# sz3/libcimbar

Hardware: NVIDIA H100
Metric: decoded cimbar frames/sec (1024x1024 mode-B) (higher is better)
Workload: dtype u8 (integer/bitwise; float32 only in the colour classifier, bit-exact vs reference)

## Files before the change

### libcimbar_b200/csrc/api.cu

```cuda
#include "ctx.cuh"
#include "k1_decode.cuh"
#include "k2_rs.cuh"
#include "render.cuh"
#include "encode.cuh"

#include <atomic>
#include <cmath>
#include <cstdio>
#include <cstring>
#include <string>
#include <vector>

using namespace cb200;

namespace {

thread_local std::string g_err;
std::atomic<unsigned long long> g_launches{0};

}
namespace cb200 {
int fail(int code, const std::string& msg) { g_err = msg; return code; }
int fail_cuda(cudaError_t e, const char* what)
{
// ... 393 lines not shown
    CK(cudaStreamCreateWithFlags(&c->own_stream, cudaStreamNonBlocking), "cudaStreamCreate");
    c->stream = c->own_stream;

    float adjust[256];
    adjust[0] = 0.0f;
    for (int d = 1; d < 256; ++d) adjust[d] = (float)(255.0 / (double)(float)d);
    unsigned long long tilesL[16];
    for (int t = 0; t < 16; ++t) tilesL[t] = brev64(kTilesH[t]);
    CK(k1_init_tables(adjust, tilesL), "k1 tables");
    CK(render_init_tables(kTilesH), "render tables");
    uint8_t gexp[512], glog[256];
    {
        unsigned el = 1; gexp[0] = 1; glog[0] = 0;
        for (unsigned i = 1; i < 512; ++i) {
            el *= 2; if (el > 255) el ^= 0x187u;
            gexp[i] = (uint8_t)el;
            if (i < 256) glog[el] = (uint8_t)i;
        }
    }
    CK(k2_init_tables(gexp, glog), "k2 tables");
    CK(flood_init_tables(adjust, tilesL, m.hash_mul), "flood tables");

    size_t n = (size_t)max_frames;
    CK(c->d_cellvals.ensure(n * m.num_cells), "cudaMalloc cellvals");
    CK(c->d_dirty.ensure(n), "cudaMalloc dirty");
    CK(c->d_raw.ensure(n * m.cap_all + 16), "cudaMalloc raw");
    CK(c->d_data.ensure(n * m.data_bytes), "cudaMalloc data");
    CK(c->d_ok.ensure(n * m.nblocks), "cudaMalloc ok");
    CK(c->d_mask.ensure(n), "cudaMalloc mask");
    CK(c->d_flags.ensure(n), "cudaMalloc flags");
    std::vector<uint16_t> idx;
    interleave_indices(m, idx);
    CK(c->d_idx.ensure(idx.size()), "cudaMalloc idx");
    CK(cudaMemcpy(c->d_idx, idx.data(), idx.size() * sizeof(uint16_t), cudaMemcpyHostToDevice), "upload idx");
    {
        std::vector<uint16_t> inv(idx.size());
        for (size_t sidx = 0; sidx < idx.size(); ++sidx) inv[idx[sidx]] = (uint16_t)sidx;
        CK(c->d_inv.ensure(inv.size()), "cudaMalloc inv");
        CK(cudaMemcpy(c->d_inv, inv.data(), inv.size() * sizeof(uint16_t), cudaMemcpyHostToDevice), "upload inv");
        std::vector<uint8_t> g(1, 1);
        auto mul = [&](uint8_t a, uint8_t b) -> uint8_t { return (a && b) ? gexp[glog[a] + glog[b]] : 0; };
        for (int i = 1; i <= m.ecc_bytes; ++i) {
            uint8_t root = gexp[i % 255];
            std::vector<uint8_t> ng(g.size() + 1, 0);
            for (size_t k = 0; k < g.size(); ++k) { ng[k + 1] ^= g[k]; ng[k] ^= mul(g[k], root); }
            g.swap(ng);
        }
        CK(c->d_gen.ensure(g.size()), "cudaMalloc gen");
        CK(cudaMemcpy(c->d_gen, g.data(), g.size(), cudaMemcpyHostToDevice), "upload gen");
        uint8_t rho[4 * 64];
        k2_remainder_basis(g.data(), m.ecc_bytes, gexp, glog, rho);
        CK(c->d_rho.ensure(sizeof(rho)), "cudaMalloc rho");
        CK(cudaMemcpy(c->d_rho, rho, sizeof(rho), cudaMemcpyHostToDevice), "upload rho");
        CK(encode_init_tables(gexp, glog), "encode tables");
    }
    {
        std::vector<uint16_t> adj;
        build_adjacency(m, adj);
        if (!adjacency_consistent(m, adj)) return fail(CB200_ERR_MODE, "adjacency self-check failed");
        CK(flood_workspace_create(m, c->sm_count, adj.data(), &c->flood), "flood workspace");
    }
    return CB200_OK;
}

int cb200_create(cb200_ctx** out, int device, int mode_val, int max_frames)
{
    if (!out || max_frames < 1) return fail(CB200_ERR_ARG, "bad arguments");
    *out = nullptr;
    int ndev = 0;
    if (cudaGetDeviceCount(&ndev) != cudaSuccess || ndev == 0)
        return fail(CB200_ERR_NODEVICE, "no CUDA device: libcb200 has no CPU fallback");
    if (device < 0) { CK(cudaGetDevice(&device), "cudaGetDevice"); }
    if (device >= ndev) return fail(CB200_ERR_ARG, "device index out of range");
    CK(cudaSetDevice(device), "cudaSetDevice");
    cb200_ctx* c = new cb200_ctx();
    c->device = device;
    int rc = create_impl(c, device, mode_val, max_frames);
    if (rc != CB200_OK) {
        std::string why = cb200_last_error();
        cb200_destroy(c);
        return fail(rc, why);
    }
    *out = c;
    return CB200_OK;
}

int cb200_destroy(cb200_ctx* c)
{
    if (!c) return CB200_OK;
    cudaSetDevice(c->device);
    for (int k = 0; k < cb200_ctx::kEvSets; ++k) for (int i = 0; i < 8; ++i) if (c->ev[k][i]) cudaEventDestroy(c->ev[k][i]);
    for (const auto& s : c->stage) if (s.ev) cudaEventDestroy(s.ev);
    if (c->ccm_ev) cudaEventDestroy(c->ccm_ev);
    gather_destroy(c->gather);
    deskew_destroy(c->deskew); scan_destroy(c->scan);
    if (c->own_stream) cudaStreamDestroy(c->own_stream);
    delete c;
    return CB200_OK;
}

int cb200_get_info(const cb200_ctx* c, cb200_info* out)
{
    if (!c || !out) return fail(CB200_ERR_ARG, "null argument");
    fill_info(c->mode, c->max_frames, c->sm_count, out);
    return CB200_OK;
}
// ... 4 lines not shown
    c->stream = cuda_stream ? (cudaStream_t)cuda_stream : c->own_stream;
    return CB200_OK;
}

int cb200_sync(cb200_ctx* c)
{
    if (!c) return fail(CB200_ERR_ARG, "null context");
    CK(cudaStreamSynchronize(c->stream), "cudaStreamSynchronize");
    return CB200_OK;
}

int cb200_decode_raw_dev(cb200_ctx* c, const uint8_t* d_rgb, int n, uint32_t flags, uint8_t* d_raw_out, uint8_t* d_frame_flags)
{
    int rc = check_frame_flags(flags); if (rc) return rc;
    rc = check_n(c, n); if (rc) return rc;
    if (n == 0) return CB200_OK;
    if (!d_rgb || !d_raw_out) return fail(CB200_ERR_ARG, "null buffer");
    CK(cudaSetDevice(c->device), "cudaSetDevice");
    const uint16_t* idx;
    rc = idx_for(c, flags, &idx); if (rc) return rc;
    rc = run_cells(c, d_rgb, n, flags, nullptr); if (rc) return rc;
    CK(k2_pack_launch(c->mode, c->d_cellvals, idx, n, d_raw_out, c->stream), "pack launch");
    mark(c);
    if (d_frame_flags) CK(cudaMemcpyAsync(d_frame_flags, c->d_flags, (size_t)n, cudaMemcpyDeviceToDevice, c->stream), "copy flags");
    return CB200_OK;
}

int cb200_rs_correct_dev(cb200_ctx* c, const uint8_t* d_raw, int n, uint8_t* d_data_out, uint8_t* d_block_ok)
{
    int rc = check_n(c, n); if (rc) return rc;
    if (n == 0) return CB200_OK;
    if (!d_raw || !d_data_out) return fail(CB200_ERR_ARG, "null buffer");
    CK(cudaSetDevice(c->device), "cudaSetDevice");
    uint8_t* ok = d_block_ok ? d_block_ok : c->d_ok;
    CK(k2_rs_launch(c->mode, d_raw, n, d_data_out, ok, c->d_rho, c->sm_count, c->stream), "rs launch");
    return CB200_OK;
}

}

namespace {
int decode_chunks(cb200_ctx* c, const uint8_t* d_rgb, int n, uint32_t flags, const uint8_t* sharpen, uint8_t* d_chunks,
                  uint32_t* d_chunk_mask, uint8_t* d_frame_flags)
{
    int rc = check_n(c, n); if (rc) return rc;
    if (n == 0) return CB200_OK;
    if (!d_rgb || !d_chunks || !d_chunk_mask) return fail(CB200_ERR_ARG, "null buffer");
    CK(cudaSetDevice(c->device), "cudaSetDevice");
    const Mode& m = c->mode;
    if ((flags & CB200_FLAG_CC_FIT) && (flags & CB200_FLAG_CC_SIMPLE)) return fail(CB200_ERR_ARG, "CC_SIMPLE and CC_FIT are exclusive");
    const bool fit = (flags & CB200_FLAG_CC_FIT) && !m.legacy && m.ecc_bytes > 0 && m.color_bits > 0;
    const uint16_t* idx;
    rc = idx_for(c, flags, &idx); if (rc) return rc;
    if (!fit) {
        rc = run_cells(c, d_rgb, n, flags & ~CB200_FLAG_CC_FIT, sharpen); if (rc) return rc;
        mark(c);
        CK(k2_rs_fused_launch(m, c->d_cellvals, idx, n, d_chunks, c->d_ok, c->d_rho, c->sm_count, c->stream), "rs launch");
    } else {
        rc = ccm_buffers(c); if (rc) return rc;
        CK(c->d_means.ensure((size_t)c->max_frames * m.num_cells), "cudaMalloc means");
        CK(c->d_ccm_active.ensure((size_t)c->max_frames), "cudaMalloc ccm flags");
        CcmArg initial;
        rc = ccm_arg(c, initial); if (rc) return rc;
        rc = run_cells(c, d_rgb, n, flags & ~(CB200_FLAG_CC_FIT | CB200_FLAG_CC_SIMPLE), sharpen, nullptr, c->d_means); if (rc) return rc;
        mark(c);
        CK(k2_rs_fused_launch(m, c->d_cellvals, idx, n, d_chunks, c->d_ok, c->d_rho, c->sm_count, c->stream, 0, m.nblocks_sym), "rs launch (symbols)");
        CK(ccm_fit_launch(m, d_rgb, d_chunks, c->d_ok, idx, n, c->d_fit, c->d_fit_valid, c->stream), "ccm fit");
        CK(ccm_carry_launch(n, c->d_fit, c->d_fit_valid, initial, c->d_ccm, c->d_ccm_active, c->stream), "ccm carry");
        CK(ccm_apply_launch(m, c->d_means, n, c->d_ccm, c->d_ccm_active, c->d_cellvals, c->stream), "ccm apply");
        CK(k2_rs_fused_launch(m, c->d_cellvals, idx, n, d_chunks, c->d_ok, c->d_rho, c->sm_count, c->stream, m.nblocks_sym, m.nblocks - m.nblocks_sym),
           "rs launch (colours)");
        rc = ccm_keep_last(c, n, c->d_ccm_active); if (rc) return rc;
    }
    mark(c);
    CK(k2_mask_launch(m, c->d_ok, n, d_chunk_mask, c->stream), "mask launch");
    mark(c);
    if (d_frame_flags) CK(cudaMemcpyAsync(d_frame_flags, c->d_flags, (size_t)n, cudaMemcpyDeviceToDevice, c->stream), "copy flags");
    return CB200_OK;
}
}

extern "C" {

int cb200_decode_chunks_dev(cb200_ctx* c, const uint8_t* d_rgb, int n, uint32_t flags, uint8_t* d_chunks, uint32_t* d_chunk_mask, uint8_t* d_frame_flags)
{
    int rc = check_frame_flags(flags); if (rc) return rc;
    return decode_chunks(c, d_rgb, n, flags, nullptr, d_chunks, d_chunk_mask, d_frame_flags);
}

int cb200_decode_chunks_sharpen_dev(cb200_ctx* c, const uint8_t* d_rgb, int n, uint32_t flags, const uint8_t* sharpen, uint8_t* d_chunks,
                                    uint32_t* d_chunk_mask, uint8_t* d_frame_flags)
{
    int rc = check_selection_args(flags, sharpen); if (rc) return rc;
    return decode_chunks(c, d_rgb, n, flags, sharpen, d_chunks, d_chunk_mask, d_frame_flags);
}

int cb200_decode_raw(cb200_ctx* c, const uint8_t* rgb, int n, uint32_t flags, uint8_t* raw_out, uint8_t* frame_flags)
{
    int rc = check_frame_flags(flags); if (rc) return rc;
    rc = check_n(c, n); if (rc) return rc;
    if (n == 0) return CB200_OK;
    if (!rgb || !raw_out) return fail(CB200_ERR_ARG, "null buffer");
    CK(cudaSetDevice(c->device), "cudaSetDevice");
    rc = upload_frames(c, rgb, n); if (rc) return rc;
    rc = cb200_decode_raw_dev(c, c->d_rgb, n, flags, c->d_raw, nullptr); if (rc) return rc;
    CK(cudaMemcpyAsync(raw_out, c->d_raw, (size_t)n * c->mode.cap_all, cudaMemcpyDeviceToHost, c->stream), "D2H raw");
    if (frame_flags) CK(cudaMemcpyAsync(frame_flags, c->d_flags, (size_t)n, cudaMemcpyDeviceToHost, c->stream), "D2H flags");
    CK(cudaStreamSynchronize(c->stream), "sync");
    return CB200_OK;
}

int cb200_decode(cb200_ctx* c, const uint8_t* rgb, int n, uint32_t flags, uint8_t* data_out, uint8_t* block_ok, uint8_t* frame_flags)
{
    int rc = check_frame_flags(flags); if (rc) return rc;
    rc = check_n(c, n); if (rc) return rc;
    if (n == 0) return CB200_OK;
    if (!rgb || !data_out) return fail(CB200_ERR_ARG, "null buffer");
    CK(cudaSetDevice(c->device), "cudaSetDevice");
    rc = upload_frames(c, rgb, n); if (rc) return rc;
    rc = cb200_decode_chunks_dev(c, c->d_rgb, n, flags, c->d_data, c->d_mask, nullptr); if (rc) return rc;
    CK(cudaMemcpyAsync(data_out, c->d_data, (size_t)n * c->mode.data_bytes, cudaMemcpyDeviceToHost, c->stream), "D2H data");
    if (block_ok) CK(cudaMemcpyAsync(block_ok, c->d_ok, (size_t)n * c->mode.nblocks, cudaMemcpyDeviceToHost, c->stream), "D2H ok");
    if (frame_flags) CK(cudaMemcpyAsync(frame_flags, c->d_flags, (size_t)n, cudaMemcpyDeviceToHost, c->stream), "D2H flags");
// ... 238 lines not shown
```

### libcimbar_b200/csrc/ctx.cuh

```cuda
#pragma once
#include "../../include/cb200.h"
#include "cb200_common.cuh"
#include "k1x_flood.cuh"
#include "ccm.cuh"

#include <string>
#include <vector>

namespace cb200 {
int fail(int code, const std::string& msg);
int fail_cuda(cudaError_t e, const char* what);
struct GatherState;
struct DeskewState;
struct ScanScratch;
void gather_destroy(GatherState* g);
void deskew_destroy(DeskewState* d);
void scan_destroy(ScanScratch* s);
int decode_fountain_to_host(cb200_ctx* c, const uint8_t* d_rgb, int n, uint32_t flags, const uint8_t* sharpen, uint8_t* chunks_out,
                            uint32_t* chunk_count, uint32_t* chunk_mask, uint8_t* frame_flags);
int check_camera_flags(uint32_t flags);
struct PicDesc {
    uint64_t src;
    uint64_t blur;
    int w, h;
    int words;
    int tile0;
};
int check_picture_sizes(const int32_t* wh, int n);
std::vector<int32_t> uniform_sizes(int w, int h, int n);
int extract_decode_to_host(cb200_ctx* c, const uint8_t* d_src, const int32_t* wh, int n, const float* corners, uint32_t flags,
                           const uint8_t* sharpen, uint8_t* chunks_out, uint32_t* chunk_count, uint32_t* chunk_mask, uint8_t* frame_flags);
std::vector<uint8_t> sharpen_from_corners(const cb200_ctx* c, const float* corners, int n);
}
#define CK(call, what) do { cudaError_t e__ = (call); if (e__ != cudaSuccess) return cb200::fail_cuda(e__, what); } while (0)

struct cb200_ctx {
    cb200::Mode mode;
    int device = 0, max_frames = 0, sm_count = 0;
    cudaStream_t own_stream = nullptr, stream = nullptr;
    cb200::DevBuf<uint8_t> d_rgb;
    cb200::DevBuf<uint8_t> d_cellvals;
    cb200::DevBuf<uint32_t> d_dirty;
    cb200::DevBuf<uint8_t> d_raw;
    cb200::DevBuf<uint8_t> d_data;
    cb200::DevBuf<uint8_t> d_ok;
    cb200::DevBuf<uint32_t> d_mask;
    cb200::DevBuf<uint8_t> d_flags;
    cb200::DevBuf<uint16_t> d_idx;
    cb200::DevBuf<uint16_t> d_inv;
    cb200::DevBuf<uint16_t> d_idx_ident;
    cb200::DevBuf<uint8_t> d_gen;
    cb200::DevBuf<uint8_t> d_rho;
    bool timing = false;
    static constexpr int kEvSets = 64;
    cudaEvent_t ev[kEvSets][8] = {};
    int ev_count[kEvSets] = {};
    long calls = 0;
    int cur = 0;
    cb200::FloodWorkspace flood;
    cb200::DevBuf<uint8_t> d_scratch;
    cb200::PinnedBuf<uint8_t> h_pinned;
    struct StageSlot { cb200::PinnedBuf<uint8_t> h; cudaEvent_t ev = nullptr; };
    static constexpr int kStageSlots = 3;
    StageSlot stage[kStageSlots];
    int stage_next = 0;
    cb200::DevBuf<uint8_t> d_sel;
    float ccm[9] = {};
    bool ccm_active = false;
    bool ccm_pending = false;
    bool ccm_pending_flag = false;
    cb200::DevBuf<float> d_ccm;
    cb200::PinnedBuf<float> h_ccm;
    cb200::DevBuf<uint32_t> d_means;
    cb200::DevBuf<float> d_fit;
    cb200::DevBuf<uint8_t> d_fit_valid;
    cb200::DevBuf<uint8_t> d_ccm_active;
    cudaEvent_t ccm_ev = nullptr;
    cb200::GatherState* gather = nullptr;
    cb200::DeskewState* deskew = nullptr;
    cb200::ScanScratch* scan = nullptr;
};

namespace cb200 {
inline void begin_timed_call(cb200_ctx* c) { if (c->timing) { c->cur = (int)(c->calls % cb200_ctx::kEvSets); c->calls++; c->ev_count[c->cur] = 0; } }
inline void mark(cb200_ctx* c) { if (c->timing && c->ev_count[c->cur] < 8) cudaEventRecord(c->ev[c->cur][c->ev_count[c->cur]++], c->stream); }
int stage_take(cb200_ctx* c, size_t bytes, int* slot, uint8_t** h);
int stage_send(cb200_ctx* c, int slot, void* d_dst, size_t bytes, const char* what);
}
```

### libcimbar_b200/csrc/k2_rs.cu

```cuda
#include "cb200_common.cuh"
#include "k2_rs.cuh"
#include <cstring>
#include <cstdint>

namespace cb200 {

constexpr int kMaxParity = 64;

__constant__ uint8_t c_gf_exp[512];
__constant__ uint8_t c_gf_log[256];

__device__ __forceinline__ uint32_t slot_value(const uint8_t* __restrict__ cells, const uint16_t* __restrict__ idx,
                                               uint32_t s, int stream, int symbol_bits)
{
    uint32_t v = cells[idx[s]] & 0x7Fu;
    uint32_t sym_mask = (1u << symbol_bits) - 1u;
    if (stream == 0) return v & sym_mask;
    if (stream == 1) return v >> symbol_bits;
    return v;
}

__device__ __forceinline__ uint32_t stream_byte(const uint8_t* __restrict__ cells, const uint16_t* __restrict__ idx,
                                                uint32_t B, int w, int stream, int symbol_bits, uint32_t nslots)
{
// ... 347 lines not shown
                }
            } else {
                const uint8_t* enc_g = raw + (size_t)f * m.cap_all + (size_t)b * blk;
                for (int i = lane; i < blk; i += 32) enc[i] = enc_g[i];
            }
        }
        __syncwarp();

        uint32_t word = 0;
        {
            const int top_src = grp * GL + (Pw - 1);
#pragma unroll 2
            for (int t = 0; t < nsteps; ++t) {
                const uint32_t ew = lds_u32(stage_lane + 4u * (uint32_t)t);
                const uint32_t tw = __shfl_sync(0xffffffffu, word, top_src);
                const uint32_t v = tw ^ __byte_perm(ew, 0u, 0x0123);
                const uint32_t r0 = lds_u32(lt_lane + (((v) & 0xFFu) + 0u) * (4u * GL));
                const uint32_t r1 = lds_u32(lt_lane + (((v >> 8) & 0xFFu) + 256u) * (4u * GL));
                const uint32_t r2 = lds_u32(lt_lane + (((v >> 16) & 0xFFu) + 512u) * (4u * GL));
                const uint32_t r3 = lds_u32(lt_lane + ((v >> 24) + 768u) * (4u * GL));
                uint32_t prev = __shfl_up_sync(0xffffffffu, word, 1, GL);
                if (k == 0) prev = 0;
                word = prev ^ r0 ^ r1 ^ r2 ^ r3;
            }
        }
        const uint32_t dirty = __ballot_sync(0xffffffffu, k < Pw && word != 0u);

#pragma unroll 1
        for (int g = 0; g < G; ++g) {
            const long gb = unit * G + g;
            if (gb >= total_blocks) break;
            const int f = (int)(gb / b_count), b = b_begin + (int)(gb - (long)f * b_count);
            uint8_t* out = data_out + ((size_t)f * m.nblocks + b) * msg_len;
            uint8_t* enc = w.stage + g * kStagePitch + lead;
            if (((dirty >> (g * GL)) & ((1u << GL) - 1u)) == 0u) {
                for (int i = lane; i < msg_len; i += 32) out[i] = enc[i];
                if (lane == 0) block_ok[(size_t)f * m.nblocks + b] = 1;
                continue;
            }
            __syncwarp();
            const bool good = rs_correct_block<T>(s, w, enc, md, blk, pad, grp == g && k < Pw, word, k, lane);
            __syncwarp();
            if (!good) {
                for (int i = lane; i < msg_len; i += 32) out[i] = 0;
                if (lane == 0) block_ok[(size_t)f * m.nblocks + b] = 0;
                continue;
            }
        for (int i = lane; i < msg_len; i += 32) out[i] = enc[i];
        if (lane == 0) block_ok[(size_t)f * m.nblocks + b] = 1;
        }
    }
}

constexpr int kFrWarps = 32;
constexpr int kFrFrames = 2;
constexpr int kFrBlk = 155, kFrWords = 39, kFrPitch = 160;

struct RsFrSmem {
    static constexpr bool kSynTable = true;
    uint8_t exp[512];
    uint8_t log[256];
    struct PerWarp {
        alignas(8) uint2 masks[32];
        alignas(4) uint8_t rem[64];
        alignas(2) uint16_t remlog[kMaxParity];
        uint8_t synd[kMaxParity];
        uint8_t loc[kMaxParity + 8];
        uint8_t last[kMaxParity + 8];
        uint8_t omega[kMaxParity];
        uint8_t roots[kMaxParity + 8];
    } w[kFrWarps];
    uint8_t la[kLaDim][kLaDim];
    alignas(8) uint2 wsyn[32][32];
};

__device__ __forceinline__ void cp_async16(uint32_t dst_shared, const void* src)
{
    asm volatile("cp.async.cg.shared.global [%0], [%1], 16;" ::"r"(dst_shared), "l"(src) : "memory");
}

__global__ void __launch_bounds__(kFrWarps * 32, 2)
k_rs_frames(const Mode m, const uint8_t* __restrict__ cellvals, const uint16_t* __restrict__ idx, int n_frames,
            uint8_t* __restrict__ data_out, uint8_t* __restrict__ block_ok, const uint8_t* __restrict__ rho, int cell_pitch)
{
    constexpr int GL = 8, G = 4;
    extern __shared__ __align__(16) uint8_t rs_smem_raw[];
    RsFrSmem& s = *reinterpret_cast<RsFrSmem*>(rs_smem_raw);
    uint8_t* dyn = rs_smem_raw + ((sizeof(RsFrSmem) + 127) & ~size_t(127));
    uint32_t* lt = reinterpret_cast<uint32_t*>(dyn);
    uint8_t* cellbuf = dyn + sizeof(uint32_t) * 4 * 256 * GL;
    uint8_t* rows = cellbuf + (size_t)kFrFrames * cell_pitch;
    const int tid = threadIdx.x, warp = tid >> 5, lane = tid & 31;
    const int md = m.ecc_bytes, msg_len = m.msg_len, nb = m.nblocks, upf = nb / G;
    const int Pw = (md + 3) >> 2, pad = 4 * Pw - md;
    const int words_per_frame = nb * kFrWords, sym_rows = m.cap_sym / kFrBlk, cell_vecs = m.num_cells >> 4;
    const bool coupled6 = m.legacy != 0;
    const int n_groups = (n_frames + kFrFrames - 1) / kFrFrames;
    const uint32_t cellbuf_s = (uint32_t)__cvta_generic_to_shared(cellbuf);

    auto load_cells = [&](int gi) {
        for (int fs = 0; fs < kFrFrames; ++fs) {
            const int f = gi * kFrFrames + fs;
            if (f >= n_frames) break;
            const uint8_t* src = cellvals + (size_t)f * m.num_cells;
            for (int i = tid; i < cell_vecs; i += (int)blockDim.x) cp_async16(cellbuf_s + (uint32_t)(fs * cell_pitch + 16 * i), src + 16 * i);
        }
        asm volatile("cp.async.commit_group;" ::: "memory");
    };
    int gi = blockIdx.x;
    if (gi < n_groups) load_cells(gi);

    for (int i = tid; i < 512; i += blockDim.x) s.exp[i] = c_gf_exp[i];
    for (int i = tid; i < 256; i += blockDim.x) s.log[i] = c_gf_log[i];
    __syncthreads();
    for (int e = tid; e < md * kLaDim; e += blockDim.x) {
        const int kk = e / kLaDim, j = e % kLaDim;
        s.la[kk][j] = (uint8_t)((255 - ((j + 1) * (md - kk)) % 255) % 255);
    }
    for (int e = tid; e < 32 * 32; e += blockDim.x) {
        const int i = e >> 5, j = e & 31;
        uint2 t = make_uint2(0u, 0u);
        if (i < md && j < md) {
            const uint32_t l = (uint32_t)((255 - ((j + 1) * (md - i)) % 255) % 255);
            t.x = (uint32_t)s.exp[l] | ((uint32_t)s.exp[l + 1] << 8) | ((uint32_t)s.exp[l + 2] << 16) | ((uint32_t)s.exp[l + 3] << 24);
            t.y = (uint32_t)s.exp[l + 4] | ((uint32_t)s.exp[l + 5] << 8) | ((uint32_t)s.exp[l + 6] << 16) | ((uint32_t)s.exp[l + 7] << 24);
        }
        s.wsyn[i][j] = t;
    }
    for (int e = tid; e < 4 * 256 * GL; e += blockDim.x) {
        const int v = e / (4 * GL), j = (e / GL) & 3, kk = e % GL;
        uint32_t word = 0;
#pragma unroll
        for (int bb = 0; bb < 4; ++bb) word |= gf_mul(s, (uint32_t)v, (uint32_t)rho[j * 64 + 4 * kk + bb]) << (8 * bb);
        lt[e] = word;
    }

    RsFrSmem::PerWarp& w = s.w[warp];
    const int grp = lane / GL, k = lane % GL;
    const uint32_t lt_lane = (uint32_t)__cvta_generic_to_shared(lt) + 4u * (uint32_t)k;
    const uint32_t vsel = 0x3210u ^ (0x1111u * (uint32_t)grp);
    const uint32_t lt0 = lt_lane + 32u * (uint32_t)(0 ^ grp), lt1 = lt_lane + 32u * (uint32_t)(1 ^ grp);
    const uint32_t lt2 = lt_lane + 32u * (uint32_t)(2 ^ grp), lt3 = lt_lane + 32u * (uint32_t)(3 ^ grp);

    for (; gi < n_groups; gi += gridDim.x) {
        asm volatile("cp.async.wait_all;" ::: "memory");
        __syncthreads();
        const int nf = (n_frames - gi * kFrFrames) < kFrFrames ? (n_frames - gi * kFrFrames) : kFrFrames;

        for (int wi = tid; wi < nf * words_per_frame; wi += (int)blockDim.x) {
            const int fs = wi >= words_per_frame ? 1 : 0;
            const int rem = wi - fs * words_per_frame;
            const int r = rem / kFrWords, q = rem - r * kFrWords;
            const uint8_t* cb = cellbuf + fs * cell_pitch;
            uint32_t b0, b1, b2, b3;
            if (coupled6) {
                auto byte6 = [&](const int B) -> uint32_t {
                    const uint32_t bit0 = 8u * (uint32_t)B, sl = bit0 / 6u, skip = bit0 - 6u * sl;
                    const uint32_t v0 = cb[idx[sl]] & 63u, v1 = cb[idx[sl + 1]] & 63u;
                    return (((v0 << 6) | v1) >> (4u - skip)) & 0xFFu;
                };
                const int B0 = r * kFrBlk + 4 * q - 1;
                b0 = q ? byte6(B0) : 0u; b1 = byte6(B0 + 1); b2 = byte6(B0 + 2); b3 = byte6(B0 + 3);
            } else if (r < sym_rows) {
                const uint32_t* ix = reinterpret_cast<const uint32_t*>(idx) + (r * kFrBlk + 4 * q);
                const uint32_t i0 = q ? ix[-1] : ix[0], i1 = ix[0], i2 = ix[1], i3 = ix[2];
                b0 = ((cb[i0 & 0xFFFFu] & 15u) << 4) | (cb[i0 >> 16] & 15u);
                b1 = ((cb[i1 & 0xFFFFu] & 15u) << 4) | (cb[i1 >> 16] & 15u);
                b2 = ((cb[i2 & 0xFFFFu] & 15u) << 4) | (cb[i2 >> 16] & 15u);
                b3 = ((cb[i3 & 0xFFFFu] & 15u) << 4) | (cb[i3 >> 16] & 15u);
            } else {
                const uint2* ix = reinterpret_cast<const uint2*>(idx) + ((r - sym_rows) * kFrBlk + 4 * q);
                const uint2 i0 = q ? ix[-1] : ix[0], i1 = ix[0], i2 = ix[1], i3 = ix[2];
                auto pack = [&](const uint2 ii) {
                    return (((uint32_t)cb[ii.x & 0xFFFFu] >> 4) & 3u) << 6 | (((uint32_t)cb[ii.x >> 16] >> 4) & 3u) << 4 |
                           (((uint32_t)cb[ii.y & 0xFFFFu] >> 4) & 3u) << 2 | (((uint32_t)cb[ii.y >> 16] >> 4) & 3u);
                };
                b0 = pack(i0); b1 = pack(i1); b2 = pack(i2); b3 = pack(i3);
            }
            if (q == 0) b0 = 0;
            *reinterpret_cast<uint32_t*>(rows + (size_t)(fs * nb + r) * kFrPitch + 4 * q) = b0 | (b1 << 8) | (b2 << 16) | (b3 << 24);
        }
        __syncthreads();
        if (gi + (int)gridDim.x < n_groups) load_cells(gi + (int)gridDim.x);

        if (warp >= nf * upf) continue;
        const int fs = warp >= upf ? 1 : 0, u = warp - fs * upf, f = gi * kFrFrames + fs;
        uint8_t* urow = rows + (size_t)(fs * nb + G * u) * kFrPitch;

        uint32_t word = 0;
        {
            const uint32_t stage_lane = (uint32_t)__cvta_generic_to_shared(urow) + (uint32_t)(grp * kFrPitch);
            const int top_src = grp * GL + (Pw - 1);
#pragma unroll 3
            for (int t = 0; t < kFrWords; ++t) {
                const uint32_t ew = lds_u32(stage_lane + 4u * (uint32_t)t);
                const uint32_t tw = __shfl_sync(0xffffffffu, word, top_src);
                const uint32_t v = __byte_perm(tw ^ __byte_perm(ew, 0u, 0x0123), 0u, vsel);
                const uint32_t r0 = lds_u32(lt0 + ((v) & 0xFFu) * 128u);
                const uint32_t r1 = lds_u32(lt1 + ((v >> 8) & 0xFFu) * 128u);
                const uint32_t r2 = lds_u32(lt2 + ((v >> 16) & 0xFFu) * 128u);
                const uint32_t r3 = lds_u32(lt3 + (v >> 24) * 128u);
                uint32_t prev = __shfl_up_sync(0xffffffffu, word, 1, GL);
                if (k == 0) prev = 0;
                word = prev ^ r0 ^ r1 ^ r2 ^ r3;
            }
        }
        const uint32_t dirty = __ballot_sync(0xffffffffu, k < Pw && word != 0u);
        uint32_t okflags = 0x01010101u;
        if (dirty) {
#pragma unroll 1
            for (int g = 0; g < G; ++g) {
                if (((dirty >> (g * GL)) & ((1u << GL) - 1u)) == 0u) continue;
                uint8_t* enc = urow + g * kFrPitch + 1;
                __syncwarp();
                const bool good = rs_correct_block<1>(s, w, enc, md, kFrBlk, pad, grp == g && k < Pw, word, k, lane);
                __syncwarp();
                if (!good) {
                    for (int i = lane; i < msg_len; i += 32) enc[i] = 0;
                    okflags &= ~(1u << (8 * g));
                }
            }
            __syncwarp();
        }
        uint32_t* out32 = reinterpret_cast<uint32_t*>(data_out + ((size_t)f * nb + (size_t)(G * u)) * msg_len);
        const uint32_t urow_s = (uint32_t)__cvta_generic_to_shared(urow);
        for (int wq = lane; wq < msg_len; wq += 32) {
            const int B = 4 * wq;
            int g = (B >= msg_len) + (B >= 2 * msg_len) + (B >= 3 * msg_len);
            int i = B - g * msg_len;
            uint32_t val;
            if (i + 4 <= msg_len) {
                const uint32_t a = (uint32_t)(g * kFrPitch + 1 + i);
                const uint32_t w0 = lds_u32(urow_s + (a & ~3u)), w1 = lds_u32(urow_s + (a & ~3u) + 4u);
                val = __funnelshift_r(w0, w1, 8u * (a & 3u));
            } else {
                val = 0;
#pragma unroll
                for (int j = 0; j < 4; ++j) {
                    val |= (uint32_t)urow[g * kFrPitch + 1 + i] << (8 * j);
                    if (++i == msg_len) { i = 0; ++g; }
                }
            }
            out32[wq] = val;
// ... 10 lines not shown
    uint32_t out = 0;
    bool carry = false;
    for (int q = 0; q < m.chunks_per_frame; ++q) {
        bool all = true;
        for (int k = 0; k < m.blocks_per_chunk; ++k) all = all && (ok[q * m.blocks_per_chunk + k] != 0);
        if (all && !carry) out |= 1u << q;
        carry = ok[q * m.blocks_per_chunk + m.blocks_per_chunk - 1] == 0;
    }
    mask[f] = out;
}

cudaError_t k2_init_tables(const uint8_t* exp512, const uint8_t* log256)
{
    cudaError_t e = cudaMemcpyToSymbol(c_gf_exp, exp512, 512);
    if (e != cudaSuccess) return e;
    return cudaMemcpyToSymbol(c_gf_log, log256, 256);
}

cudaError_t k2_pack_launch(const Mode& m, const uint8_t* d_cellvals, const uint16_t* d_idx, int n_frames, uint8_t* d_raw, cudaStream_t st)
{
    dim3 grid((m.cap_all + 255) / 256, n_frames);
    k_pack_raw<<<grid, 256, 0, st>>>(m, d_cellvals, d_idx, n_frames, d_raw); count_launch();
    return cudaGetLastError();
}

template <int T, bool FUSED>
static cudaError_t rs_launch_t(const Mode& m, const uint8_t* d_raw, const uint8_t* d_cellvals, const uint16_t* d_idx, int n_frames,
                               uint8_t* d_data, uint8_t* d_ok, const uint8_t* d_rho, int sm_count, cudaStream_t st, int b_begin = 0, int b_count = -1)
{
    if (b_count < 0) b_count = m.nblocks;
    if (m.ecc_block + 4 > kStagePitch || m.ecc_bytes > 8 * T * 4 || m.ecc_bytes > kLaDim) return cudaErrorInvalidValue;
    const size_t smem = ((sizeof(RsSmem<T>) + 127) & ~size_t(127)) + sizeof(uint32_t) * 4 * 256 * 8 * T;
    {
        cudaError_t e = cudaFuncSetAttribute(k_rs_decode<T, FUSED>, cudaFuncAttributeMaxDynamicSharedMemorySize, (int)smem);
        if (e != cudaSuccess) return e;
    }
    const int G = 4 / T;
    long total = (long)n_frames * b_count;
    long units = (total + G - 1) / G;
    long ctas = (units + kRsWarpsPerCta - 1) / kRsWarpsPerCta;
    long max_ctas = (long)sm_count * (T == 1 ? 4 : 2);
    if (ctas > max_ctas) ctas = max_ctas;
    if (ctas < 1) ctas = 1;
    k_rs_decode<T, FUSED><<<(int)ctas, kRsWarpsPerCta * 32, smem, st>>>(m, d_raw, d_cellvals, d_idx, n_frames, b_begin, b_count, d_data, d_ok, d_rho); count_launch();
    return cudaGetLastError();
}

cudaError_t k2_rs_launch(const Mode& m, const uint8_t* d_raw, int n_frames, uint8_t* d_data, uint8_t* d_ok, const uint8_t* d_rho, int sm_count, cudaStream_t st)
{
    if (m.ecc_bytes <= 32) return rs_launch_t<1, false>(m, d_raw, nullptr, nullptr, n_frames, d_data, d_ok, d_rho, sm_count, st);
    return rs_launch_t<2, false>(m, d_raw, nullptr, nullptr, n_frames, d_data, d_ok, d_rho, sm_count, st);
}

cudaError_t k2_rs_fused_launch(const Mode& m, const uint8_t* d_cellvals, const uint16_t* d_idx, int n_frames, uint8_t* d_data,
                               uint8_t* d_ok, const uint8_t* d_rho, int sm_count, cudaStream_t st, int b_begin, int b_count)
{
    if (b_count < 0) b_count = m.nblocks;
    const bool whole = b_begin == 0 && b_count == m.nblocks;
    const bool bits_ok = m.symbol_bits == 4 && m.color_bits == 2 && (!m.legacy || (size_t)m.num_cells * 6 == (size_t)m.cap_all * 8);
    if (whole && bits_ok && m.ecc_block == kFrBlk && m.ecc_bytes <= 32 &&
        m.ecc_bytes <= kLaDim && m.nblocks % 4 == 0 && kFrFrames * (m.nblocks / 4) <= kFrWarps && m.num_cells % 16 == 0 &&
        m.cap_sym % kFrBlk == 0 && (m.nblocks * m.msg_len) % 4 == 0 && ((uintptr_t)d_data & 3u) == 0 && n_frames > 0) {
        const int cell_pitch = m.num_cells;
        const size_t smem = ((sizeof(RsFrSmem) + 127) & ~size_t(127)) + sizeof(uint32_t) * 4 * 256 * 8 +
                            (size_t)kFrFrames * cell_pitch + (size_t)kFrFrames * m.nblocks * kFrPitch;
        if (smem <= 113 * 1024) {
            cudaError_t e = cudaFuncSetAttribute(k_rs_frames, cudaFuncAttributeMaxDynamicSharedMemorySize, (int)smem);
            if (e != cudaSuccess) return e;
            int groups = (n_frames + kFrFrames - 1) / kFrFrames, ctas = groups < 2 * sm_count ? groups : 2 * sm_count;
            k_rs_frames<<<ctas, 32 * kFrFrames * (m.nblocks / 4), smem, st>>>(m, d_cellvals, d_idx, n_frames, d_data, d_ok, d_rho, cell_pitch); count_launch();
            return cudaGetLastError();
        }
    }
    if (m.ecc_bytes <= 32) return rs_launch_t<1, true>(m, nullptr, d_cellvals, d_idx, n_frames, d_data, d_ok, d_rho, sm_count, st, b_begin, b_count);
    return rs_launch_t<2, true>(m, nullptr, d_cellvals, d_idx, n_frames, d_data, d_ok, d_rho, sm_count, st, b_begin, b_count);
}

void k2_remainder_basis(const uint8_t* gen, int parity, const uint8_t* gexp512, const uint8_t* glog256, uint8_t* rho_out )
{
    const int Pw = (parity + 3) / 4, D = 4 * Pw, pad = D - parity;
    uint8_t G[72] = {0};
    for (int k = 0; k <= parity; ++k) G[pad + k] = gen[k];
    auto mul = [&](uint8_t x, uint8_t y) -> uint8_t { return (x && y) ? gexp512[glog256[x] + glog256[y]] : 0; };
    uint8_t r[64] = {0};
    r[0] = 1;
    for (int e = 1; e <= D + 3; ++e) {
        const uint8_t top = r[D - 1];
        for (int k = D - 1; k > 0; --k) r[k] = r[k - 1];
        r[0] = 0;
        if (top) for (int k = 0; k < D; ++k) r[k] ^= mul(top, G[k]);
        if (e >= D) { for (int k = 0; k < 64; ++k) rho_out[(e - D) * 64 + k] = k < D ? r[k] : 0; }
    }
}

cudaError_t k2_mask_launch(const Mode& m, const uint8_t* d_ok, int n_frames, uint32_t* d_mask, cudaStream_t st)
{
    k_chunk_mask<<<(n_frames + 127) / 128, 128, 0, st>>>(m, d_ok, n_frames, d_mask); count_launch();
    return cudaGetLastError();
}

}
```

### libcimbar_b200/csrc/k2_rs.cuh

```cuda
#pragma once
#include "cb200_common.cuh"

namespace cb200 {
cudaError_t k2_init_tables(const uint8_t* exp512, const uint8_t* log256);
cudaError_t k2_pack_launch(const Mode& m, const uint8_t* d_cellvals, const uint16_t* d_idx, int n_frames, uint8_t* d_raw, cudaStream_t st);
cudaError_t k2_rs_launch(const Mode& m, const uint8_t* d_raw, int n_frames, uint8_t* d_data, uint8_t* d_ok, const uint8_t* d_rho, int sm_count, cudaStream_t st);
void k2_remainder_basis(const uint8_t* gen, int parity, const uint8_t* gexp512, const uint8_t* glog256, uint8_t* rho_out);
cudaError_t k2_rs_fused_launch(const Mode& m, const uint8_t* d_cellvals, const uint16_t* d_idx, int n_frames, uint8_t* d_data,
                               uint8_t* d_ok, const uint8_t* d_rho, int sm_count, cudaStream_t st, int b_begin = 0, int b_count = -1);
cudaError_t k2_mask_launch(const Mode& m, const uint8_t* d_ok, int n_frames, uint32_t* d_mask, cudaStream_t st);
}
```

Before: 901,600.

## Replace per-byte index gather with analytic interleave unpack in fused RS kernel

```diff
diff --git a/libcimbar_b200/csrc/api.cu b/libcimbar_b200/csrc/api.cu
--- a/libcimbar_b200/csrc/api.cu
+++ b/libcimbar_b200/csrc/api.cu
@@ -469,6 +469,10 @@
         k2_remainder_basis(g.data(), m.ecc_bytes, gexp, glog, rho);
         CK(c->d_rho.ensure(sizeof(rho)), "cudaMalloc rho");
         CK(cudaMemcpy(c->d_rho, rho, sizeof(rho), cudaMemcpyHostToDevice), "upload rho");
+        std::vector<uint64_t> tables((k2_frame_tables_size() + 7) / 8);
+        k2_frame_tables(gexp, glog, rho, m.ecc_bytes, tables.data());
+        CK(c->d_rs_tables.ensure(k2_frame_tables_size()), "cudaMalloc rs tables");
+        CK(cudaMemcpy(c->d_rs_tables, tables.data(), k2_frame_tables_size(), cudaMemcpyHostToDevice), "upload rs tables");
         CK(encode_init_tables(gexp, glog), "encode tables");
     }
     {
@@ -579,10 +583,11 @@
     const bool fit = (flags & CB200_FLAG_CC_FIT) && !m.legacy && m.ecc_bytes > 0 && m.color_bits > 0;
     const uint16_t* idx;
     rc = idx_for(c, flags, &idx); if (rc) return rc;
+    const bool il = !(flags & CB200_FLAG_NO_INTERLEAVE);
     if (!fit) {
         rc = run_cells(c, d_rgb, n, flags & ~CB200_FLAG_CC_FIT, sharpen); if (rc) return rc;
         mark(c);
-        CK(k2_rs_fused_launch(m, c->d_cellvals, idx, n, d_chunks, c->d_ok, c->d_rho, c->sm_count, c->stream), "rs launch");
+        CK(k2_rs_fused_launch(m, c->d_cellvals, idx, il, n, d_chunks, c->d_ok, c->d_rho, c->d_rs_tables, c->sm_count, c->stream), "rs launch");
     } else {
         rc = ccm_buffers(c); if (rc) return rc;
         CK(c->d_means.ensure((size_t)c->max_frames * m.num_cells), "cudaMalloc means");
@@ -591,11 +596,12 @@
         rc = ccm_arg(c, initial); if (rc) return rc;
         rc = run_cells(c, d_rgb, n, flags & ~(CB200_FLAG_CC_FIT | CB200_FLAG_CC_SIMPLE), sharpen, nullptr, c->d_means); if (rc) return rc;
         mark(c);
-        CK(k2_rs_fused_launch(m, c->d_cellvals, idx, n, d_chunks, c->d_ok, c->d_rho, c->sm_count, c->stream, 0, m.nblocks_sym), "rs launch (symbols)");
+        CK(k2_rs_fused_launch(m, c->d_cellvals, idx, il, n, d_chunks, c->d_ok, c->d_rho, c->d_rs_tables, c->sm_count, c->stream, 0, m.nblocks_sym), "rs launch (symbols)");
         CK(ccm_fit_launch(m, d_rgb, d_chunks, c->d_ok, idx, n, c->d_fit, c->d_fit_valid, c->stream), "ccm fit");
         CK(ccm_carry_launch(n, c->d_fit, c->d_fit_valid, initial, c->d_ccm, c->d_ccm_active, c->stream), "ccm carry");
         CK(ccm_apply_launch(m, c->d_means, n, c->d_ccm, c->d_ccm_active, c->d_cellvals, c->stream), "ccm apply");
-        CK(k2_rs_fused_launch(m, c->d_cellvals, idx, n, d_chunks, c->d_ok, c->d_rho, c->sm_count, c->stream, m.nblocks_sym, m.nblocks - m.nblocks_sym),
+        CK(k2_rs_fused_launch(m, c->d_cellvals, idx, il, n, d_chunks, c->d_ok, c->d_rho, c->d_rs_tables, c->sm_count, c->stream, m.nblocks_sym,
+                              m.nblocks - m.nblocks_sym),
            "rs launch (colours)");
         rc = ccm_keep_last(c, n, c->d_ccm_active); if (rc) return rc;
     }
diff --git a/libcimbar_b200/csrc/ctx.cuh b/libcimbar_b200/csrc/ctx.cuh
--- a/libcimbar_b200/csrc/ctx.cuh
+++ b/libcimbar_b200/csrc/ctx.cuh
@@ -51,6 +51,7 @@
     cb200::DevBuf<uint16_t> d_idx_ident;
     cb200::DevBuf<uint8_t> d_gen;
     cb200::DevBuf<uint8_t> d_rho;
+    cb200::DevBuf<uint8_t> d_rs_tables;
     bool timing = false;
     static constexpr int kEvSets = 64;
     cudaEvent_t ev[kEvSets][8] = {};
diff --git a/libcimbar_b200/csrc/k2_rs.cu b/libcimbar_b200/csrc/k2_rs.cu
--- a/libcimbar_b200/csrc/k2_rs.cu
+++ b/libcimbar_b200/csrc/k2_rs.cu
@@ -423,143 +423,183 @@
     }
 }
 
-constexpr int kFrWarps = 32;
-constexpr int kFrFrames = 2;
+constexpr int kFrWarps = 16;
 constexpr int kFrBlk = 155, kFrWords = 39, kFrPitch = 160;
-
-struct RsFrSmem {
-    static constexpr bool kSynTable = true;
+constexpr int kFrLead = 16;
+
+struct RsFrTables {
     uint8_t exp[512];
     uint8_t log[256];
+    alignas(8) uint2 wsyn[32][32];
+    uint32_t lt[4 * 256 * 8];
+};
+static_assert(sizeof(RsFrTables) % 16 == 0, "the tables are copied in 16-byte pieces");
+
+struct RsFrSmem : RsFrTables {
+    static constexpr bool kSynTable = true;
     struct PerWarp {
         alignas(8) uint2 masks[32];
         alignas(4) uint8_t rem[64];
-        alignas(2) uint16_t remlog[kMaxParity];
         uint8_t synd[kMaxParity];
         uint8_t loc[kMaxParity + 8];
         uint8_t last[kMaxParity + 8];
         uint8_t omega[kMaxParity];
         uint8_t roots[kMaxParity + 8];
     } w[kFrWarps];
-    uint8_t la[kLaDim][kLaDim];
-    alignas(8) uint2 wsyn[32][32];
 };
 
+__host__ __device__ inline int fr_cell_pitch(const Mode& m) { return (m.num_cells + 31) & ~15; }
+__host__ __device__ inline int fr_stream_pitch(const Mode& m) { return (kFrLead + m.cap_all + 8 + 15) & ~15; }
+__host__ __device__ inline int fr_tasks(const Mode& m, int part, int rows)
+{
+    return rows == 1 ? (m.num_cells + 31) >> 5 : (m.num_cells / part) * (rows >> 3) * ((part / rows + 3) >> 2);
+}
+
 __device__ __forceinline__ void cp_async16(uint32_t dst_shared, const void* src)
 {
     asm volatile("cp.async.cg.shared.global [%0], [%1], 16;" ::"r"(dst_shared), "l"(src) : "memory");
 }
 
 __global__ void __launch_bounds__(kFrWarps * 32, 2)
-k_rs_frames(const Mode m, const uint8_t* __restrict__ cellvals, const uint16_t* __restrict__ idx, int n_frames,
-            uint8_t* __restrict__ data_out, uint8_t* __restrict__ block_ok, const uint8_t* __restrict__ rho, int cell_pitch)
+k_rs_frames(const Mode m, const uint8_t* __restrict__ cellvals, int n_frames, int part, int rows, uint8_t* __restrict__ data_out,
+            uint8_t* __restrict__ block_ok, const RsFrTables* __restrict__ tables)
 {
     constexpr int GL = 8, G = 4;
     extern __shared__ __align__(16) uint8_t rs_smem_raw[];
     RsFrSmem& s = *reinterpret_cast<RsFrSmem*>(rs_smem_raw);
-    uint8_t* dyn = rs_smem_raw + ((sizeof(RsFrSmem) + 127) & ~size_t(127));
-    uint32_t* lt = reinterpret_cast<uint32_t*>(dyn);
-    uint8_t* cellbuf = dyn + sizeof(uint32_t) * 4 * 256 * GL;
-    uint8_t* rows = cellbuf + (size_t)kFrFrames * cell_pitch;
+    const int cell_pitch = fr_cell_pitch(m);
+    uint8_t* cellbuf = rs_smem_raw + ((sizeof(RsFrSmem) + 127) & ~size_t(127));
+    uint8_t* stream = cellbuf + 2 * cell_pitch + kFrLead;
+    uint8_t* rows_b = cellbuf + 2 * cell_pitch + fr_stream_pitch(m);
+    const uint32_t cells_s = (uint32_t)__cvta_generic_to_shared(cellbuf);
     const int tid = threadIdx.x, warp = tid >> 5, lane = tid & 31;
-    const int md = m.ecc_bytes, msg_len = m.msg_len, nb = m.nblocks, upf = nb / G;
+    const int md = m.ecc_bytes, msg_len = m.msg_len, nb = m.nblocks;
     const int Pw = (md + 3) >> 2, pad = 4 * Pw - md;
-    const int words_per_frame = nb * kFrWords, sym_rows = m.cap_sym / kFrBlk, cell_vecs = m.num_cells >> 4;
+    const int cell_vecs = m.num_cells >> 4;
     const bool coupled6 = m.legacy != 0;
-    const int n_groups = (n_frames + kFrFrames - 1) / kFrFrames;
-    const uint32_t cellbuf_s = (uint32_t)__cvta_generic_to_shared(cellbuf);
-
-    auto load_cells = [&](int gi) {
-        for (int fs = 0; fs < kFrFrames; ++fs) {
-            const int f = gi * kFrFrames + fs;
-            if (f >= n_frames) break;
+
+    auto load_cells = [&](int f, int buf) {
+        if (f < n_frames) {
             const uint8_t* src = cellvals + (size_t)f * m.num_cells;
-            for (int i = tid; i < cell_vecs; i += (int)blockDim.x) cp_async16(cellbuf_s + (uint32_t)(fs * cell_pitch + 16 * i), src + 16 * i);
+            for (int i = tid; i < cell_vecs; i += (int)blockDim.x) cp_async16(cells_s + (uint32_t)(buf * cell_pitch + 16 * i), src + 16 * i);
         }
         asm volatile("cp.async.commit_group;" ::: "memory");
     };
-    int gi = blockIdx.x;
-    if (gi < n_groups) load_cells(gi);
-
-    for (int i = tid; i < 512; i += blockDim.x) s.exp[i] = c_gf_exp[i];
-    for (int i = tid; i < 256; i += blockDim.x) s.log[i] = c_gf_log[i];
-    __syncthreads();
-    for (int e = tid; e < md * kLaDim; e += blockDim.x) {
-        const int kk = e / kLaDim, j = e % kLaDim;
-        s.la[kk][j] = (uint8_t)((255 - ((j + 1) * (md - kk)) % 255) % 255);
-    }
-    for (int e = tid; e < 32 * 32; e += blockDim.x) {
-        const int i = e >> 5, j = e & 31;
-        uint2 t = make_uint2(0u, 0u);
-        if (i < md && j < md) {
-            const uint32_t l = (uint32_t)((255 - ((j + 1) * (md - i)) % 255) % 255);
-            t.x = (uint32_t)s.exp[l] | ((uint32_t)s.exp[l + 1] << 8) | ((uint32_t)s.exp[l + 2] << 16) | ((uint32_t)s.exp[l + 3] << 24);
-            t.y = (uint32_t)s.exp[l + 4] | ((uint32_t)s.exp[l + 5] << 8) | ((uint32_t)s.exp[l + 6] << 16) | ((uint32_t)s.exp[l + 7] << 24);
-        }
-        s.wsyn[i][j] = t;
-    }
-    for (int e = tid; e < 4 * 256 * GL; e += blockDim.x) {
-        const int v = e / (4 * GL), j = (e / GL) & 3, kk = e % GL;
-        uint32_t word = 0;
-#pragma unroll
-        for (int bb = 0; bb < 4; ++bb) word |= gf_mul(s, (uint32_t)v, (uint32_t)rho[j * 64 + 4 * kk + bb]) << (8 * bb);
-        lt[e] = word;
-    }
-
-    RsFrSmem::PerWarp& w = s.w[warp];
-    const int grp = lane / GL, k = lane % GL;
-    const uint32_t lt_lane = (uint32_t)__cvta_generic_to_shared(lt) + 4u * (uint32_t)k;
-    const uint32_t vsel = 0x3210u ^ (0x1111u * (uint32_t)grp);
-    const uint32_t lt0 = lt_lane + 32u * (uint32_t)(0 ^ grp), lt1 = lt_lane + 32u * (uint32_t)(1 ^ grp);
-    const uint32_t lt2 = lt_lane + 32u * (uint32_t)(2 ^ grp), lt3 = lt_lane + 32u * (uint32_t)(3 ^ grp);
-
-    for (; gi < n_groups; gi += gridDim.x) {
-        asm volatile("cp.async.wait_all;" ::: "memory");
+    {
+        const uint32_t tab_s = (uint32_t)__cvta_generic_to_shared(&s);
+        const uint8_t* tab = reinterpret_cast<const uint8_t*>(tables);
+        for (int i = tid; i < (int)(sizeof(RsFrTables) / 16); i += (int)blockDim.x) cp_async16(tab_s + 16u * (uint32_t)i, tab + 16 * i);
+    }
+    load_cells(blockIdx.x, 0);
+    load_cells(blockIdx.x + gridDim.x, 1);
+
+    const int task = tid, ntasks = fr_tasks(m, part, rows);
+    int cell0 = 0, slot0 = 0, run_step = 8, nruns = 0, rot = 0, cols = part / rows;
+    if (task < ntasks) {
+        if (rows == 1) {
+            cell0 = slot0 = 32 * task;
+            nruns = (m.num_cells - slot0) >> 3;
+            rot = (task >> 3) & 3;
+        } else {
+            const int cgs = (cols + 3) >> 2, per_part = (rows >> 3) * cgs;
+            const int p = task / per_part, rg = (task - p * per_part) / cgs, cg = task - p * per_part - rg * cgs;
+            cell0 = p * part + 8 * rg * cols + 4 * cg;
+            slot0 = p * part + 4 * cg * rows + 8 * rg;
+            run_step = rows;
+            nruns = cols - 4 * cg;
+            rot = (cg >> 3) & 3;
+        }
+        if (nruns > 4) nruns = 4;
+    }
+
+    for (int it = 0, f = blockIdx.x; f < n_frames; ++it, f += gridDim.x) {
+        const int buf = it & 1;
+        asm volatile("cp.async.wait_group 1;" ::: "memory");
         __syncthreads();
-        const int nf = (n_frames - gi * kFrFrames) < kFrFrames ? (n_frames - gi * kFrFrames) : kFrFrames;
-
-        for (int wi = tid; wi < nf * words_per_frame; wi += (int)blockDim.x) {
-            const int fs = wi >= words_per_frame ? 1 : 0;
-            const int rem = wi - fs * words_per_frame;
-            const int r = rem / kFrWords, q = rem - r * kFrWords;
-            const uint8_t* cb = cellbuf + fs * cell_pitch;
-            uint32_t b0, b1, b2, b3;
-            if (coupled6) {
-                auto byte6 = [&](const int B) -> uint32_t {
-                    const uint32_t bit0 = 8u * (uint32_t)B, sl = bit0 / 6u, skip = bit0 - 6u * sl;
-                    const uint32_t v0 = cb[idx[sl]] & 63u, v1 = cb[idx[sl + 1]] & 63u;
-                    return (((v0 << 6) | v1) >> (4u - skip)) & 0xFFu;
-                };
-                const int B0 = r * kFrBlk + 4 * q - 1;
-                b0 = q ? byte6(B0) : 0u; b1 = byte6(B0 + 1); b2 = byte6(B0 + 2); b3 = byte6(B0 + 3);
-            } else if (r < sym_rows) {
-                const uint32_t* ix = reinterpret_cast<const uint32_t*>(idx) + (r * kFrBlk + 4 * q);
-                const uint32_t i0 = q ? ix[-1] : ix[0], i1 = ix[0], i2 = ix[1], i3 = ix[2];
-                b0 = ((cb[i0 & 0xFFFFu] & 15u) << 4) | (cb[i0 >> 16] & 15u);
-                b1 = ((cb[i1 & 0xFFFFu] & 15u) << 4) | (cb[i1 >> 16] & 15u);
-                b2 = ((cb[i2 & 0xFFFFu] & 15u) << 4) | (cb[i2 >> 16] & 15u);
-                b3 = ((cb[i3 & 0xFFFFu] & 15u) << 4) | (cb[i3 >> 16] & 15u);
+
+        if (task < ntasks) {
+            const uint8_t* cb = cellbuf + buf * cell_pitch;
+            uint32_t R[8];
+            if (rows == 1) {
+                const uint4 x = *reinterpret_cast<const uint4*>(cb + cell0), y = *reinterpret_cast<const uint4*>(cb + cell0 + 16);
+                const uint32_t W[8] = {x.x, x.y, x.z, x.w, y.x, y.y, y.z, y.w};
+#pragma unroll
+                for (int i = 0; i < 8; ++i) {
+                    const uint32_t sel = (uint32_t)(i & 3) | ((uint32_t)(4 + (i & 3)) << 4);
+                    R[i] = __byte_perm(__byte_perm(W[i >> 2], W[2 + (i >> 2)], sel), __byte_perm(W[4 + (i >> 2)], W[6 + (i >> 2)], sel), 0x5410);
+                }
             } else {
-                const uint2* ix = reinterpret_cast<const uint2*>(idx) + ((r - sym_rows) * kFrBlk + 4 * q);
-                const uint2 i0 = q ? ix[-1] : ix[0], i1 = ix[0], i2 = ix[1], i3 = ix[2];
-                auto pack = [&](const uint2 ii) {
-                    return (((uint32_t)cb[ii.x & 0xFFFFu] >> 4) & 3u) << 6 | (((uint32_t)cb[ii.x >> 16] >> 4) & 3u) << 4 |
-                           (((uint32_t)cb[ii.y & 0xFFFFu] >> 4) & 3u) << 2 | (((uint32_t)cb[ii.y >> 16] >> 4) & 3u);
-                };
-                b0 = pack(i0); b1 = pack(i1); b2 = pack(i2); b3 = pack(i3);
-            }
-            if (q == 0) b0 = 0;
-            *reinterpret_cast<uint32_t*>(rows + (size_t)(fs * nb + r) * kFrPitch + 4 * q) = b0 | (b1 << 8) | (b2 << 16) | (b3 << 24);
+#pragma unroll
+                for (int i = 0; i < 8; ++i) {
+                    const uint32_t o = (uint32_t)(cell0 + i * cols);
+                    const uint32_t* a = reinterpret_cast<const uint32_t*>(cb + (o & ~3u));
+                    R[i] = __funnelshift_r(a[0], a[1], 8u * (o & 3u));
+                }
+            }
+            const uint32_t n4 = 0x0F0F0F0Fu, n2 = 0x03030303u;
+            if (!coupled6) {
+                uint32_t P[4], Q[2];
+#pragma unroll
+                for (int k = 0; k < 4; ++k) P[k] = ((R[2 * k] & n4) << 4) | (R[2 * k + 1] & n4);
+#pragma unroll
+                for (int k = 0; k < 2; ++k)
+                    Q[k] = (((R[4 * k] >> 4) & n2) << 6) | (((R[4 * k + 1] >> 4) & n2) << 4) | (((R[4 * k + 2] >> 4) & n2) << 2) | ((R[4 * k + 3] >> 4) & n2);
+#pragma unroll
+                for (int jj = 0; jj < 4; ++jj) {
+                    const int j = (jj + rot) & 3;
+                    if (j < nruns) {
+                        const uint32_t sel = (uint32_t)j | ((uint32_t)(4 + j) << 4), S = (uint32_t)(slot0 + j * run_step);
+                        *reinterpret_cast<uint32_t*>(stream + S / 2u) = __byte_perm(__byte_perm(P[0], P[1], sel), __byte_perm(P[2], P[3], sel), 0x5410);
+                        *reinterpret_cast<uint16_t*>(stream + m.cap_sym + S / 4u) = (uint16_t)__byte_perm(Q[0], Q[1], sel);
+                    }
+                }
+            } else {
+                uint32_t B[6];
+#pragma unroll
+                for (int h = 0; h < 2; ++h) {
+                    const uint32_t v0 = R[4 * h] & 0x3F3F3F3Fu, v1 = R[4 * h + 1] & 0x3F3F3F3Fu, v2 = R[4 * h + 2] & 0x3F3F3F3Fu,
+                                   v3 = R[4 * h + 3] & 0x3F3F3F3Fu;
+                    B[3 * h] = (v0 << 2) | ((v1 >> 4) & n2);
+                    B[3 * h + 1] = ((v1 & n4) << 4) | ((v2 >> 2) & n4);
+                    B[3 * h + 2] = ((v2 & n2) << 6) | v3;
+                }
+#pragma unroll
+                for (int jj = 0; jj < 4; ++jj) {
+                    const int j = (jj + rot) & 3;
+                    if (j < nruns) {
+                        const uint32_t sel = (uint32_t)j | ((uint32_t)(4 + j) << 4);
+                        uint16_t* a = reinterpret_cast<uint16_t*>(stream + 3u * (uint32_t)(slot0 + j * run_step) / 4u);
+                        a[0] = (uint16_t)__byte_perm(B[0], B[1], sel);
+                        a[1] = (uint16_t)__byte_perm(B[2], B[3], sel);
+                        a[2] = (uint16_t)__byte_perm(B[4], B[5], sel);
+                    }
+                }
+            }
         }
         __syncthreads();
-        if (gi + (int)gridDim.x < n_groups) load_cells(gi + (int)gridDim.x);
-
-        if (warp >= nf * upf) continue;
-        const int fs = warp >= upf ? 1 : 0, u = warp - fs * upf, f = gi * kFrFrames + fs;
-        uint8_t* urow = rows + (size_t)(fs * nb + G * u) * kFrPitch;
+        load_cells(f + 2 * (int)gridDim.x, buf);
+
+        for (int wi = tid; wi < nb * kFrWords; wi += (int)blockDim.x) {
+            const int r = wi / kFrWords, q = wi - r * kFrWords;
+            const uint32_t o = (uint32_t)(r * kFrBlk + 4 * q - 1 + kFrLead);
+            const uint32_t* a = reinterpret_cast<const uint32_t*>(stream - kFrLead + (o & ~3u));
+            uint32_t v = __funnelshift_r(a[0], a[1], 8u * (o & 3u));
+            if (q == 0) v &= 0xFFFFFF00u;
+            *reinterpret_cast<uint32_t*>(rows_b + r * kFrPitch + 4 * q) = v;
+        }
+        __syncthreads();
+
+        const int u = warp;
+        uint8_t* urow = rows_b + (size_t)(G * u) * kFrPitch;
+        RsFrSmem::PerWarp& w = s.w[warp];
+        const int grp = lane / GL, k = lane % GL;
 
         uint32_t word = 0;
         {
+            const uint32_t lt_lane = (uint32_t)__cvta_generic_to_shared(s.lt) + 4u * (uint32_t)k;
+            const uint32_t vsel = 0x3210u ^ (0x1111u * (uint32_t)grp);
+            const uint32_t lt0 = lt_lane + 32u * (uint32_t)(0 ^ grp), lt1 = lt_lane + 32u * (uint32_t)(1 ^ grp);
+            const uint32_t lt2 = lt_lane + 32u * (uint32_t)(2 ^ grp), lt3 = lt_lane + 32u * (uint32_t)(3 ^ grp);
             const uint32_t stage_lane = (uint32_t)__cvta_generic_to_shared(urow) + (uint32_t)(grp * kFrPitch);
             const int top_src = grp * GL + (Pw - 1);
 #pragma unroll 3
@@ -676,28 +716,57 @@
     return rs_launch_t<2, false>(m, d_raw, nullptr, nullptr, n_frames, d_data, d_ok, d_rho, sm_count, st);
 }
 
-cudaError_t k2_rs_fused_launch(const Mode& m, const uint8_t* d_cellvals, const uint16_t* d_idx, int n_frames, uint8_t* d_data,
-                               uint8_t* d_ok, const uint8_t* d_rho, int sm_count, cudaStream_t st, int b_begin, int b_count)
+cudaError_t k2_rs_fused_launch(const Mode& m, const uint8_t* d_cellvals, const uint16_t* d_idx, bool interleaved, int n_frames,
+                               uint8_t* d_data, uint8_t* d_ok, const uint8_t* d_rho, const void* d_frame_tables, int sm_count,
+                               cudaStream_t st, int b_begin, int b_count)
 {
     if (b_count < 0) b_count = m.nblocks;
     const bool whole = b_begin == 0 && b_count == m.nblocks;
     const bool bits_ok = m.symbol_bits == 4 && m.color_bits == 2 && (!m.legacy || (size_t)m.num_cells * 6 == (size_t)m.cap_all * 8);
-    if (whole && bits_ok && m.ecc_block == kFrBlk && m.ecc_bytes <= 32 &&
-        m.ecc_bytes <= kLaDim && m.nblocks % 4 == 0 && kFrFrames * (m.nblocks / 4) <= kFrWarps && m.num_cells % 16 == 0 &&
-        m.cap_sym % kFrBlk == 0 && (m.nblocks * m.msg_len) % 4 == 0 && ((uintptr_t)d_data & 3u) == 0 && n_frames > 0) {
-        const int cell_pitch = m.num_cells;
-        const size_t smem = ((sizeof(RsFrSmem) + 127) & ~size_t(127)) + sizeof(uint32_t) * 4 * 256 * 8 +
-                            (size_t)kFrFrames * cell_pitch + (size_t)kFrFrames * m.nblocks * kFrPitch;
+    const int part = m.num_cells / 2, rows = interleaved ? part / m.ecc_block : 1;
+    const bool map_ok = m.num_cells % 2 == 0 && part % m.ecc_block == 0 && part % 8 == 0 && (rows == 1 || rows % 8 == 0);
+    const int warps = m.nblocks / 4;
+    if (whole && bits_ok && map_ok && m.ecc_block == kFrBlk && m.ecc_bytes <= 32 && m.nblocks % 4 == 0 && warps <= kFrWarps &&
+        fr_tasks(m, part, rows) <= 32 * warps && m.num_cells % 16 == 0 && m.cap_sym % kFrBlk == 0 && (m.nblocks * m.msg_len) % 4 == 0 &&
+        ((uintptr_t)d_data & 3u) == 0 && n_frames > 0) {
+        const size_t smem = ((sizeof(RsFrSmem) + 127) & ~size_t(127)) + 2 * (size_t)fr_cell_pitch(m) + (size_t)fr_stream_pitch(m) +
+                            (size_t)m.nblocks * kFrPitch;
         if (smem <= 113 * 1024) {
             cudaError_t e = cudaFuncSetAttribute(k_rs_frames, cudaFuncAttributeMaxDynamicSharedMemorySize, (int)smem);
             if (e != cudaSuccess) return e;
-            int groups = (n_frames + kFrFrames - 1) / kFrFrames, ctas = groups < 2 * sm_count ? groups : 2 * sm_count;
-            k_rs_frames<<<ctas, 32 * kFrFrames * (m.nblocks / 4), smem, st>>>(m, d_cellvals, d_idx, n_frames, d_data, d_ok, d_rho, cell_pitch); count_launch();
+            const int ctas = n_frames < 2 * sm_count ? n_frames : 2 * sm_count;
+            k_rs_frames<<<ctas, 32 * warps, smem, st>>>(m, d_cellvals, n_frames, part, rows, d_data, d_ok,
+                                                        static_cast<const RsFrTables*>(d_frame_tables)); count_launch();
             return cudaGetLastError();
         }
     }
     if (m.ecc_bytes <= 32) return rs_launch_t<1, true>(m, nullptr, d_cellvals, d_idx, n_frames, d_data, d_ok, d_rho, sm_count, st, b_begin, b_count);
     return rs_launch_t<2, true>(m, nullptr, d_cellvals, d_idx, n_frames, d_data, d_ok, d_rho, sm_count, st, b_begin, b_count);
+}
+
+size_t k2_frame_tables_size() { return sizeof(RsFrTables); }
+
+void k2_frame_tables(const uint8_t* gexp512, const uint8_t* glog256, const uint8_t* rho, int parity, void* out)
+{
+    RsFrTables& t = *static_cast<RsFrTables*>(out);
+    memcpy(t.exp, gexp512, 512);
+    memcpy(t.log, glog256, 256);
+    auto mul = [&](uint32_t x, uint32_t y) -> uint32_t { return (x && y) ? gexp512[glog256[x] + glog256[y]] : 0u; };
+    for (int i = 0; i < 32; ++i)
+        for (int j = 0; j < 32; ++j) {
+            uint2 w = make_uint2(0u, 0u);
+            if (i < parity && j < parity) {
+                const int l = (255 - ((j + 1) * (parity - i)) % 255) % 255;
+                for (int b = 0; b < 4; ++b) { w.x |= (uint32_t)gexp512[l + b] << (8 * b); w.y |= (uint32_t)gexp512[l + 4 + b] << (8 * b); }
+            }
+            t.wsyn[i][j] = w;
+        }
+    for (int e = 0; e < 4 * 256 * 8; ++e) {
+        const int v = e / 32, j = (e / 8) & 3, kk = e % 8;
+        uint32_t word = 0;
+        for (int bb = 0; bb < 4; ++bb) word |= mul((uint32_t)v, rho[j * 64 + 4 * kk + bb]) << (8 * bb);
+        t.lt[e] = word;
+    }
 }
 
 void k2_remainder_basis(const uint8_t* gen, int parity, const uint8_t* gexp512, const uint8_t* glog256, uint8_t* rho_out )
diff --git a/libcimbar_b200/csrc/k2_rs.cuh b/libcimbar_b200/csrc/k2_rs.cuh
--- a/libcimbar_b200/csrc/k2_rs.cuh
+++ b/libcimbar_b200/csrc/k2_rs.cuh
@@ -6,7 +6,10 @@
 cudaError_t k2_pack_launch(const Mode& m, const uint8_t* d_cellvals, const uint16_t* d_idx, int n_frames, uint8_t* d_raw, cudaStream_t st);
 cudaError_t k2_rs_launch(const Mode& m, const uint8_t* d_raw, int n_frames, uint8_t* d_data, uint8_t* d_ok, const uint8_t* d_rho, int sm_count, cudaStream_t st);
 void k2_remainder_basis(const uint8_t* gen, int parity, const uint8_t* gexp512, const uint8_t* glog256, uint8_t* rho_out);
-cudaError_t k2_rs_fused_launch(const Mode& m, const uint8_t* d_cellvals, const uint16_t* d_idx, int n_frames, uint8_t* d_data,
-                               uint8_t* d_ok, const uint8_t* d_rho, int sm_count, cudaStream_t st, int b_begin = 0, int b_count = -1);
+size_t k2_frame_tables_size();
+void k2_frame_tables(const uint8_t* gexp512, const uint8_t* glog256, const uint8_t* rho, int parity, void* out);
+cudaError_t k2_rs_fused_launch(const Mode& m, const uint8_t* d_cellvals, const uint16_t* d_idx, bool interleaved, int n_frames,
+                               uint8_t* d_data, uint8_t* d_ok, const uint8_t* d_rho, const void* d_frame_tables, int sm_count,
+                               cudaStream_t st, int b_begin = 0, int b_count = -1);
 cudaError_t k2_mask_launch(const Mode& m, const uint8_t* d_ok, int n_frames, uint32_t* d_mask, cudaStream_t st);
 }
```

Result: no change. 909,500, median of 6 (+0.9%).
